# bcaitech1/p4-fr-sorry-math-but-love-you

Measured on NVIDIA B200. Metric: EfficientSATRN greedy-decode images/sec, higher is better.
Workload: dtype bf16

## Files before the change

p4-fr-sorry-math-but-love-you_b200/csrc/kernels_decode_bf16.cu:

```cuda
#include <cooperative_groups.h>
#include <cstdio>
#include <cstdlib>

#include "common.cuh"
#include "kernels.h"

namespace cg = cooperative_groups;

namespace frx {

namespace {

#ifndef FRX_DEC_D
#define FRX_DEC_D 256
#define FRX_DEC_FF 1024
#define FRX_DEC_NAME(x) x
#endif
#ifndef FRX_DEC_HPC
#define FRX_DEC_HPC 1
#endif
#ifndef FRX_DEC_HD
#define FRX_DEC_HD 32
#endif
constexpr int D = FRX_DEC_D;
// ... 136 lines not shown
      mma_bf16(acc[j][1], a1, wk[j].z, wk[j].w);
    }
  };
  if constexpr (C::TOT <= 16) {
    uint4 w[C::TOT];
#pragma unroll
    for (int idx = 0; idx < C::TOT; ++idx) {
      const int kk = idx / C::TPW, j = idx % C::TPW;
      if (idx < PF) w[idx] = pre.w[idx];
      else w[idx] = wload(kk, j);
    }
#pragma unroll
    for (int kk = 0; kk < C::KPW; ++kk) kstep(kk, &w[kk * C::TPW]);
  } else {
    static_assert(PF == 0 || PF == C::TPW, "streaming stages prefetch exactly their first k-pair");
    constexpr int RING = 3;
    uint4 w[RING][C::TPW];
#pragma unroll
    for (int r = 0; r < RING - 1; ++r)
#pragma unroll
      for (int j = 0; j < C::TPW; ++j) {
        if (r < C::KPW) w[r][j] = (PF > 0 && r == 0) ? pre.w[j] : wload(r, j);
      }
#pragma unroll
    for (int kk = 0; kk < C::KPW; ++kk) {
      if (kk + RING - 1 < C::KPW) {
#pragma unroll
        for (int j = 0; j < C::TPW; ++j) w[(kk + RING - 1) % RING][j] = wload(kk + RING - 1, j);
      }
      kstep(kk, w[kk % RING]);
    }
  }
#pragma unroll
  for (int j = 0; j < C::TPW; ++j)
    *reinterpret_cast<float2*>(red + ((size_t)(ks * NT + tg + j * C::TG) * 32 + lane) * 2) =
        make_float2(acc[j][0][0] + acc[j][1][0], acc[j][0][1] + acc[j][1][1]);
  __syncthreads();
  if (threadIdx.x < C::UNITS * C::NSUB) {
    const int u = threadIdx.x % C::UNITS, sub = threadIdx.x / C::UNITS;
    const int tile = u >> 3, row = u & 7;
    float v[8];
#pragma unroll
    for (int i = 0; i < 8; ++i) v[i] = 0.f;
#pragma unroll
    for (int k2 = 0; k2 < KS; ++k2) {
      const float4* src = reinterpret_cast<const float4*>(red + ((size_t)(k2 * NT + tile) * 32 + row * 4) * 2);
      const float4 lo = src[0], hi = src[1];
      v[0] += lo.x; v[1] += lo.y; v[2] += lo.z; v[3] += lo.w;
      v[4] += hi.x; v[5] += hi.y; v[6] += hi.z; v[7] += hi.w;
    }
    epi(tile, row, v, sub);
  }
}

__device__ __forceinline__ uint32_t mapa_u32(uint32_t addr, uint32_t rank) {
  uint32_t r;
  asm volatile("mapa.shared::cluster.u32 %0, %1, %2;\n" : "=r"(r) : "r"(addr), "r"(rank));
  return r;
}
__device__ __forceinline__ void st_async_b32(uint32_t raddr, uint32_t v, uint32_t rbar) {
  asm volatile("st.async.weak.shared::cluster.mbarrier::complete_tx::bytes.b32 [%0], %1, [%2];\n" ::"r"(raddr), "r"(v), "r"(rbar) : "memory");
}
__device__ __forceinline__ void st_async_v4(uint32_t raddr, uint4 v, uint32_t rbar) {
  asm volatile("st.async.weak.shared::cluster.mbarrier::complete_tx::bytes.v4.b32 [%0], {%1, %2, %3, %4}, [%5];\n" ::"r"(raddr), "r"(v.x), "r"(v.y), "r"(v.z), "r"(v.w), "r"(rbar) : "memory");
}
__device__ __forceinline__ void mbar_init(uint32_t bar, uint32_t count) {
  asm volatile("mbarrier.init.shared::cta.b64 [%0], %1;\n" ::"r"(bar), "r"(count) : "memory");
}
__device__ __forceinline__ void mbar_expect_tx(uint32_t bar, uint32_t bytes) {
  asm volatile("mbarrier.arrive.expect_tx.shared::cta.b64 _, [%0], %1;\n" ::"r"(bar), "r"(bytes) : "memory");
}
__device__ __forceinline__ void mbar_wait(uint32_t bar, uint32_t parity) {
  uint32_t ok = 0;
#ifndef FRX_DEC_SPINLIMIT
#define FRX_DEC_SPINLIMIT (1ll << 26)
#endif
#pragma unroll 1
  for (long long spins = 0; spins < FRX_DEC_SPINLIMIT; ++spins) {
    asm volatile(
        "{\n"
        ".reg .pred p;\n"
        "mbarrier.try_wait.parity.shared::cta.b64 p, [%1], %2;\n"
        "selp.u32 %0, 1, 0, p;\n"
        "}\n" : "=r"(ok) : "r"(bar), "r"(parity) : "memory");
    if (ok) return;
  }
  __trap();
}


struct LnParams { float g[D / 32], b[D / 32]; };
__device__ __forceinline__ LnParams load_ln(const float* __restrict__ g, const float* __restrict__ b) {
  LnParams o;
  const int lane = threadIdx.x & 31;
#pragma unroll
  for (int i = 0; i < D / 32; ++i) { o.g[i] = __ldg(g + i * 32 + lane); o.b[i] = __ldg(b + i * 32 + lane); }
  return o;
}

__device__ __forceinline__ void layernorm_rows(Smem& s, const LnParams& P) {
  const int row = threadIdx.x >> 5, lane = threadIdx.x & 31;
  if (row >= NIMG) return;
  float v[D / 32];
#pragma unroll
  for (int i = 0; i < D / 32; ++i) v[i] = s.pre[row][i * 32 + lane];
  const float shift = __shfl_sync(0xffffffffu, v[0], 0);
  float s1 = 0.f, s2 = 0.f;
#pragma unroll
  for (int i = 0; i < D / 32; ++i) { const float d = v[i] - shift; s1 += d; s2 = fmaf(d, d, s2); }
#pragma unroll
  for (int o = 16; o > 0; o >>= 1) {
    s1 += __shfl_xor_sync(0xffffffffu, s1, o);
    s2 += __shfl_xor_sync(0xffffffffu, s2, o);
  }
  const float md = s1 * (1.f / D);
  const float mean = shift + md;
  const float rstd = rsqrtf(fmaxf(s2 * (1.f / D) - md * md, 0.f) + 1e-5f);
#pragma unroll
  for (int i = 0; i < D / 32; ++i) {
    const int c = i * 32 + lane;
    const float o = (v[i] - mean) * rstd * P.g[i] + P.b[i];
    s.xres[row][c] = o;
    s.abf[row][c] = __float2bfloat16_rn(o);
  }
}

struct KVStage { __nv_bfloat16 k[32][HD], v[32][HD]; };

__device__ __forceinline__ int kv_perm(int row) {
  if constexpr (HD == 32) return (row >> 1) & 3;
  else return row & (HD / 8 - 1);
}
__device__ __forceinline__ uint32_t kv_swz(int row, int chunk) { return (uint32_t)(row * (HD * 2) + ((chunk ^ kv_perm(row)) << 4)); }

__device__ __forceinline__ void kv_request(KVStage& st, const __nv_bfloat16* __restrict__ Kc, const __nv_bfloat16* __restrict__ Vc,
                                           int kb, int n_hist, const int* __restrict__ chain) {
  if (kb < n_hist) {
    const int lane = threadIdx.x & 31;
    const uint32_t ks = smem_u32(&st.k[0][0]), vs = smem_u32(&st.v[0][0]);
#pragma unroll
    for (int i = 0; i < HD / 8; ++i) {
      const int id = lane + 32 * i, row = id / (HD / 8), chunk = id % (HD / 8);
      const int key = kb + row;
      const uint32_t bytes = key < n_hist ? 16u : 0u;
      int src = key < n_hist ? key : 0;
      if (chain) src = __ldg(chain + src);
      const size_t off = (size_t)src * HD + ((chunk ^ kv_perm(src)) << 3);
      asm volatile("cp.async.cg.shared.global [%0], [%1], 16, %2;\n" ::"r"(ks + kv_swz(row, chunk)), "l"(Kc + off), "r"(bytes) : "memory");
      asm volatile("cp.async.cg.shared.global [%0], [%1], 16, %2;\n" ::"r"(vs + kv_swz(row, chunk)), "l"(Vc + off), "r"(bytes) : "memory");
    }
  }
  asm volatile("cp.async.commit_group;\n" ::: "memory");
}
__device__ __forceinline__ void kv_request_bulk(KVStage& st, uint32_t bar, const __nv_bfloat16* __restrict__ Kc,
                                                const __nv_bfloat16* __restrict__ Vc, int kb, int n_hist) {
  if (kb < n_hist && (threadIdx.x & 31) == 0) {
    const int rows = n_hist - kb < 32 ? n_hist - kb : 32;
    const uint32_t bytes = (uint32_t)rows * (HD * 2);
    asm volatile("mbarrier.arrive.expect_tx.shared::cta.b64 _, [%0], %1;\n" ::"r"(bar), "r"(2u * bytes) : "memory");
    asm volatile("cp.async.bulk.shared::cluster.global.mbarrier::complete_tx::bytes [%0], [%1], %2, [%3];\n"
                 ::"r"(smem_u32(&st.k[0][0])), "l"(Kc + (size_t)kb * HD), "r"(bytes), "r"(bar) : "memory");
    asm volatile("cp.async.bulk.shared::cluster.global.mbarrier::complete_tx::bytes [%0], [%1], %2, [%3];\n"
                 ::"r"(smem_u32(&st.v[0][0])), "l"(Vc + (size_t)kb * HD), "r"(bytes), "r"(bar) : "memory");
  }
}
__device__ __forceinline__ void kv_prime(KVStage* ring, const __nv_bfloat16* __restrict__ Kc, const __nv_bfloat16* __restrict__ Vc, int n_hist,
                                         const int* __restrict__ chain, uint32_t kvbar) {
  if (!KV_BULK || chain) {
#pragma unroll
    for (int d = 0; d < KVD; ++d) kv_request(ring[d], Kc, Vc, 32 * d, n_hist, chain);
  } else {
#pragma unroll
    for (int d = 0; d < KVD; ++d) kv_request_bulk(ring[d], kvbar + 8u * d, Kc, Vc, 32 * d, n_hist);
  }
}

__device__ __forceinline__ float ex2f(float x) {
  float y;
  asm("ex2.approx.ftz.f32 %0, %1;\n" : "=f"(y) : "f"(x));
  return y;
}

template <bool BULK>
__device__ __forceinline__ void attend_mma(KVStage* ring, const float* __restrict__ q, const __nv_bfloat16* __restrict__ Kc,
                                           const __nv_bfloat16* __restrict__ Vc, int n_hist, const int* __restrict__ chain,
                                           uint32_t kvbar, uint32_t& kvphase, const __nv_bfloat16* __restrict__ kx,
                                           const __nv_bfloat16* __restrict__ vx, float qscale,
                                           float (&o)[HD / 4], long long* pw = nullptr) {
  constexpr int NK = HD / 16;
  constexpr int ND = HD / 8;
  const int lane = threadIdx.x & 31, tig = lane & 3;
  uint32_t aq[NK][4];
#pragma unroll
  for (int ks = 0; ks < NK; ++ks) {
    const float2 qa = *reinterpret_cast<const float2*>(q + 16 * ks + 2 * tig), qb = *reinterpret_cast<const float2*>(q + 16 * ks + 8 + 2 * tig);
    aq[ks][0] = pack_bf16(qa.x * qscale, qa.y * qscale); aq[ks][1] = 0u;
    aq[ks][2] = pack_bf16(qb.x * qscale, qb.y * qscale); aq[ks][3] = 0u;
  }
  float m = -INFINITY, l = 0.f;
  float acc[ND][4];
#pragma unroll
  for (int nt = 0; nt < ND; ++nt)
#pragma unroll
    for (int e = 0; e < 4; ++e) acc[nt][e] = 0.f;
  const int lrow = lane & 7, lmat = lane >> 3;
  uint32_t koff[ND / 4], voff[ND / 2];
#pragma unroll
  for (int c4 = 0; c4 < ND / 4; ++c4) koff[c4] = kv_swz(lrow, 4 * c4 + lmat);
#pragma unroll
  for (int np = 0; np < ND / 2; ++np) voff[np] = kv_swz((lmat & 1) * 8 + lrow, 2 * np + (lmat >> 1));
  int slot = 0;
  for (int kb = 0; kb < n_hist; kb += 32) {
    KVStage& st = ring[slot];
    const int cur = slot;
    slot = slot + 1 == KVD ? 0 : slot + 1;
    const uint32_t ks = smem_u32(&st.k[0][0]), vs = smem_u32(&st.v[0][0]);
    long long tw = 0;
    if (pw) tw = clock64();
    if (!BULK) {
      asm volatile("cp.async.wait_group %0;\n" ::"n"(KVD - 1) : "memory");
    } else {
      mbar_wait(kvbar + 8u * cur, (kvphase >> cur) & 1u);
      kvphase ^= 1u << cur;
    }
    if (pw) { const long long tn = clock64(); pw[0] += tn - tw; pw[1] += 1; tw = tn; }
    __syncwarp();
    uint32_t kf[4][ND], vf[2][ND / 2][4];
#pragma unroll
    for (int j = 0; j < 4; ++j)
#pragma unroll
      for (int c4 = 0; c4 < ND / 4; ++c4)
        asm volatile("ldmatrix.sync.aligned.m8n8.x4.shared.b16 {%0,%1,%2,%3}, [%4];\n"
                     : "=r"(kf[j][4 * c4 + 0]), "=r"(kf[j][4 * c4 + 1]), "=r"(kf[j][4 * c4 + 2]), "=r"(kf[j][4 * c4 + 3])
                     : "r"(ks + koff[c4] + (uint32_t)(j * 8 * HD * 2)));
#pragma unroll
    for (int ks2 = 0; ks2 < 2; ++ks2)
#pragma unroll
      for (int np = 0; np < ND / 2; ++np)
        asm volatile("ldmatrix.sync.aligned.m8n8.x4.trans.shared.b16 {%0,%1,%2,%3}, [%4];\n"
                     : "=r"(vf[ks2][np][0]), "=r"(vf[ks2][np][1]), "=r"(vf[ks2][np][2]), "=r"(vf[ks2][np][3])
                     : "r"(vs + voff[np] + (uint32_t)(ks2 * 16 * HD * 2)));
    __syncwarp();
    if (!BULK) kv_request(st, Kc, Vc, kb + 32 * KVD, n_hist, chain);
    else kv_request_bulk(st, kvbar + 8u * cur, Kc, Vc, kb + 32 * KVD, n_hist);
    if (pw) { const long long tn = clock64(); pw[2] += tn - tw; tw = tn; }
    float sc[4][4];
#pragma unroll
    for (int j = 0; j < 4; ++j) {
#pragma unroll
      for (int e = 0; e < 4; ++e) sc[j][e] = 0.f;
#pragma unroll
      for (int k2 = 0; k2 < NK; ++k2) mma_bf16(sc[j], aq[k2], kf[j][2 * k2], kf[j][2 * k2 + 1]);
    }
    if (!BULK || kb + 32 > n_hist) {
#pragma unroll
      for (int j = 0; j < 4; ++j)
#pragma unroll
        for (int e = 0; e < 2; ++e)
          if (kb + 8 * j + 2 * tig + e >= n_hist) sc[j][e] = -INFINITY;
    }
    float cm = fmaxf(fmaxf(fmaxf(sc[0][0], sc[0][1]), fmaxf(sc[1][0], sc[1][1])), fmaxf(fmaxf(sc[2][0], sc[2][1]), fmaxf(sc[3][0], sc[3][1])));
    cm = fmaxf(cm, __shfl_xor_sync(0xffffffffu, cm, 1));
    cm = fmaxf(cm, __shfl_xor_sync(0xffffffffu, cm, 2));
    cm = fmaxf(cm, m);
    if (!BULK || cm > m) {
      const float scale = ex2f(m - cm);
      m = cm;
      l *= scale;
#pragma unroll
      for (int nt = 0; nt < ND; ++nt) { acc[nt][0] *= scale; acc[nt][1] *= scale; }
    }
    if (pw) { const long long tn = clock64(); pw[3] += tn - tw; tw = tn; }
    float pr[4][2];
#pragma unroll
    for (int j = 0; j < 4; ++j)
#pragma unroll
      for (int e = 0; e < 2; ++e) pr[j][e] = ex2f(sc[j][e] - m);
    l += ((pr[0][0] + pr[0][1]) + (pr[1][0] + pr[1][1])) + ((pr[2][0] + pr[2][1]) + (pr[3][0] + pr[3][1]));
#pragma unroll
    for (int ks2 = 0; ks2 < 2; ++ks2) {
      const uint32_t ap[4] = {pack_bf16(pr[2 * ks2][0], pr[2 * ks2][1]), 0u, pack_bf16(pr[2 * ks2 + 1][0], pr[2 * ks2 + 1][1]), 0u};
#pragma unroll
      for (int np = 0; np < ND / 2; ++np) {
        mma_bf16(acc[2 * np], ap, vf[ks2][np][0], vf[ks2][np][1]);
        mma_bf16(acc[2 * np + 1], ap, vf[ks2][np][2], vf[ks2][np][3]);
      }
    }
    if (pw) pw[4] += clock64() - tw;
  }
  l += __shfl_xor_sync(0xffffffffu, l, 1);
  l += __shfl_xor_sync(0xffffffffu, l, 2);
  if (kx) {
    constexpr int DPT = HD / 4;
    float part = 0.f;
#pragma unroll
    for (int c8 = 0; c8 < DPT / 8; ++c8) {
      const float4 q0 = *reinterpret_cast<const float4*>(q + DPT * tig + 8 * c8), q1 = *reinterpret_cast<const float4*>(q + DPT * tig + 8 * c8 + 4);
      float kf[8];
      unpack8(*reinterpret_cast<const uint4*>(kx + DPT * tig + 8 * c8), kf);
      part += q0.x * kf[0] + q0.y * kf[1] + q0.z * kf[2] + q0.w * kf[3] + q1.x * kf[4] + q1.y * kf[5] + q1.z * kf[6] + q1.w * kf[7];
    }
    part += __shfl_xor_sync(0xffffffffu, part, 1);
    part += __shfl_xor_sync(0xffffffffu, part, 2);
    const float s_cur = part * qscale;
    const float M = fmaxf(m, s_cur);
    const float gs = ex2f(m - M);
    const float pc = ex2f(s_cur - M);
    l = l * gs + pc;
#pragma unroll
    for (int nt = 0; nt < ND; ++nt) {
      const __nv_bfloat162 v2 = *reinterpret_cast<const __nv_bfloat162*>(vx + 8 * nt + 2 * tig);
      acc[nt][0] = fmaf(pc, __low2float(v2), acc[nt][0] * gs);
      acc[nt][1] = fmaf(pc, __high2float(v2), acc[nt][1] * gs);
    }
  }
  const float inv = __fdividef(1.f, l);
#pragma unroll
  for (int nt = 0; nt < ND; ++nt) { o[2 * nt] = acc[nt][0] * inv; o[2 * nt + 1] = acc[nt][1] * inv; }
}

__device__ __forceinline__ float4 ldg4(const float* p) { return __ldg(reinterpret_cast<const float4*>(p)); }

__device__ __noinline__ int sift_pick(const float* lrow, int V, int4* state, const int* __restrict__ flags, const int* __restrict__ limit,
                                      SiftIds ids, float* prow) {
  const int lane = threadIdx.x & 31;
  const int4 stt = *state;
  float mx = -INFINITY;
  for (int i = lane; i < V; i += 32) mx = fmaxf(mx, lrow[i]);
#pragma unroll
  for (int o = 16; o > 0; o >>= 1) mx = fmaxf(mx, __shfl_xor_sync(0xffffffffu, mx, o));
  float sum = 0.f;
  for (int i = lane; i < V; i += 32) sum += expf(lrow[i] - mx);
#pragma unroll
  for (int o = 16; o > 0; o >>= 1) sum += __shfl_xor_sync(0xffffffffu, sum, o);
  const int cur = stt.x;
  const int cf = (cur >= 0 && cur < V) ? __ldg(flags + cur) : 0;
  const int clim = (cur >= 0 && cur < V) ? __ldg(limit + cur) : 0;
  float best = -INFINITY;
  int bi = 0x7fffffff;
  for (int i = lane; i < V; i += 32) {
    bool black = (i == ids.sos) || (i == ids.empty) || (i == ids.rbrace && stt.z == stt.w);
    if (cur == ids.eos) {
    } else if (cur == ids.sos) {
      black = black || (__ldg(flags + i) & 1);
    } else if (cf & 2) {
      black = black || (i != ids.underbar);
    } else if (cf & 4) {
      black = black || (i != ids.lbrace);
    } else {
      if ((cf & 8) && i == ids.underbar) black = true;
      if ((cf & 16) && i == ids.lbrace) black = true;
      if (clim > 0 && stt.y >= clim && i == cur) black = true;
    }
    const float pv = black ? 0.f : expf(lrow[i] - mx) / sum;
    if (prow) prow[i] = pv;
    if (pv > best) { best = pv; bi = i; }
  }
#pragma unroll
  for (int o = 16; o > 0; o >>= 1) {
    const float ob = __shfl_xor_sync(0xffffffffu, best, o);
    const int oi = __shfl_xor_sync(0xffffffffu, bi, o);
    if (ob > best || (ob == best && oi < bi)) { best = ob; bi = oi; }
  }
  if (bi < 0 || bi >= V) bi = 0;
  __syncwarp();
  if (lane == 0) {
    int4 n = stt;
    n.y = (bi == stt.x) ? stt.y + 1 : 1;
    if (bi == ids.lbrace) n.z += 1;
    else if (bi == ids.rbrace) n.w += 1;
    n.x = bi;
    *state = n;
  }
  __syncwarp();
  return bi;
}
struct Bias8 { float4 a, b; };
__device__ __forceinline__ Bias8 ldg_bias8(const float* p, bool active) {
  Bias8 o;
  o.a = o.b = make_float4(0.f, 0.f, 0.f, 0.f);
  if (active) { o.a = ldg4(p); o.b = ldg4(p + 4); }
  return o;
}

}

#ifndef FRX_DEC_MINBLOCKS
#define FRX_DEC_MINBLOCKS (NTHR <= 256 ? 2 : 1)
#endif
__global__ void __cluster_dims__(CL, 1, 1) __launch_bounds__(NTHR, FRX_DEC_MINBLOCKS)
FRX_DEC_NAME(dec_cluster_bf16_kernel)(const DecClusterP p) {
  extern __shared__ __align__(16) unsigned char smem_raw[];
  Smem& s = *reinterpret_cast<Smem*>(smem_raw);
  cg::cluster_group cl = cg::this_cluster();
  const int r = (int)cl.block_rank();
  const int img0 = p.img_base + (blockIdx.x / CL) * NIMG;
  const int tid = threadIdx.x, warp = tid >> 5, lane = tid & 31;
  const uint64_t pol = make_evict_last_policy();
  const float qscale = 1.4426950408889634f / sqrtf((float)D);
  const float emb_scale = sqrtf((float)D);
  const int L = p.L, T = p.T, V = p.V, B = p.B;
  constexpr int LDA = D + APAD, LDA2 = FF + APAD;
  constexpr int KPD = D / 32, KPF = FF / 32;
  constexpr size_t WT = (size_t)KPD * 32;
  constexpr int KS = 2;
  constexpr int PF_A = GC<NTA, KPD, KS>::TOT > 16 ? GC<NTA, KPD, KS>::TPW : (GC<NTA, KPD, KS>::TOT < 6 ? GC<NTA, KPD, KS>::TOT : 6);
  constexpr int PF_S = GC<NTS, KPD, KS>::TOT;
  constexpr int PF_E = GC<NTE, KPD, KS>::TOT < 8 ? GC<NTE, KPD, KS>::TOT : 8;
  constexpr int PF_F = GC<NTS, KPF, KS>::TOT < 8 ? GC<NTS, KPF, KS>::TOT : 8;

  if (tid == 0) {
#pragma unroll
    for (int l = 0; l < 4; ++l) s.lw[l] = p.layer[l];
  }
  for (int i = tid; i < NIMG * D; i += NTHR) {
    const int row = i / D, c = i % D;
    const int b = min(img0 + row, p.B - 1);
    long long tok = p.sos;
    if (p.first_tok32) tok = __ldg(p.first_tok32 + b);
    else if (p.first_tok64) tok = __ldg(p.first_tok64 + b);
    const int pos0 = p.hist_len ? __ldg(p.hist_len + b) : 0;
    float v = __ldg(p.emb + (size_t)tok * D + c) * emb_scale + __ldg(p.pe + (size_t)pos0 * D + c);
    s.xres[row][c] = v;
    s.abf[row][c] = __float2bfloat16_rn(v);
  }
  if (tid < NIMG) s.sift[tid] = make_int4(p.sift_ids.sos, 1, 0, 0);
  const uint32_t bar0 = smem_u32(&s.bar[0]), bar1 = smem_u32(&s.bar[1]);
  if (tid == 0) {
    mbar_init(bar0, 1);
    mbar_init(bar1, 1);
    asm volatile("fence.mbarrier_init.release.cluster;\n" ::: "memory");
  }
  if (KV_BULK) {
    if (lane == 0) {
#pragma unroll
      for (int d = 0; d < KVD; ++d) mbar_init(smem_u32(&s.kvbar[warp][d]), 1);
    }
    for (int i = tid; i < (int)(sizeof(s.kvst) / 16); i += NTHR) reinterpret_cast<uint4*>(&s.kvst[0][0][0][0][0])[i] = make_uint4(0u, 0u, 0u, 0u);
    asm volatile("fence.proxy.async.shared::cta;\n" ::: "memory");
  }
  __syncthreads();
  cl.sync();
  int gstage = 0;
  auto stage_bar = [&]() -> uint32_t { return (gstage & 1) ? bar1 : bar0; };
  auto stage_begin = [&](uint32_t bytes) { if (tid == 0) mbar_expect_tx(stage_bar(), bytes); };
  auto stage_end = [&]() { mbar_wait(stage_bar(), (uint32_t)((gstage >> 1) & 1)); ++gstage; };
  int rsel = 0;
  auto next_red = [&]() -> float* { rsel ^= 1; return s.red[rsel]; };
  float* const logit_s = reinterpret_cast<float*>(&s.abf2[0][0]);
  constexpr int LGS = VP + FPAD;
  static_assert(NIMG * LGS * 4 <= NIMG * (FF + APAD) * 2, "the fp32 logits view must fit in abf2");

  const bool profiling = p.prof != nullptr && blockIdx.x == 0 && tid == 0;
  if (profiling) for (int i = 0; i < 16; ++i) s.prof[i] = 0;
  long long tprev = clock64();
  auto mark = [&](int id) {
    if (profiling) {
      long long now = clock64();
      s.prof[id] += now - tprev;
      tprev = now;
    }
  };
  const int wimg = warp % NIMG, whc = warp / NIMG;
  const int head = r * HPC + whc;
  const int b_mine = img0 + wimg;
  const bool mine = b_mine < B;
  const int hist0 = (mine && p.hist_len) ? __ldg(p.hist_len + b_mine) : 0;
  const int* const chain = (mine && p.chain) ? p.chain + (size_t)b_mine * T : nullptr;
  KVStage* const kvst = reinterpret_cast<KVStage*>(&s.kvst[warp][0][0][0][0]);
  const uint32_t kvbar = smem_u32(&s.kvbar[warp][0]);
  uint32_t kvphase = 0;

  auto store_attn = [&](uint32_t sb, const float (&o)[HD / 4]) {
    const uint32_t dst = (uint32_t)(lane >> 2);
    if (dst < (uint32_t)CL) {
      const uint32_t rb = mapa_u32(sb, dst);
      const uint32_t la = mapa_u32(smem_u32(&s.obf[wimg][head * HD + 2 * (lane & 3)]), dst);
#pragma unroll
      for (int nt = 0; nt < HD / 8; ++nt) st_async_b32(la + nt * 16, pack_bf16(o[2 * nt], o[2 * nt + 1]), rb);
    }
  };
  auto pre_bias = [&](const float* bias) {
    return ldg_bias8(bias + r * SW + ((tid % (NTS * 8)) >> 3) * 8, true);
  };
  auto pre_epi = [&](uint32_t sb, const Bias8& bias, bool relu) {
    return [&, sb, bias, relu](int tile, int row, float (&v)[8], int sub) {
      constexpr int NSUB_S = GC<NTS, KPD, KS>::NSUB, DPT = (CL + NSUB_S - 1) / NSUB_S;
      if (sub * DPT >= CL) return;
      const int col = r * SW + tile * 8;
      const float4 b0 = bias.a, b1 = bias.b;
      const float4 x0 = *reinterpret_cast<const float4*>(&s.xres[row][col]), x1 = *reinterpret_cast<const float4*>(&s.xres[row][col + 4]);
      float o[8] = {v[0] + b0.x, v[1] + b0.y, v[2] + b0.z, v[3] + b0.w, v[4] + b1.x, v[5] + b1.y, v[6] + b1.z, v[7] + b1.w};
      if (relu) {
#pragma unroll
        for (int i = 0; i < 8; ++i) o[i] = fmaxf(o[i], 0.f);
      }
      const uint4 lo = make_uint4(__float_as_uint(o[0] + x0.x), __float_as_uint(o[1] + x0.y), __float_as_uint(o[2] + x0.z), __float_as_uint(o[3] + x0.w));
      const uint4 hi = make_uint4(__float_as_uint(o[4] + x1.x), __float_as_uint(o[5] + x1.y), __float_as_uint(o[6] + x1.z), __float_as_uint(o[7] + x1.w));
#pragma unroll
      for (int d = 0; d < DPT; ++d) {
        const uint32_t dst = (uint32_t)(sub * DPT + d);
        if (dst >= (uint32_t)CL) break;
        const uint32_t la = mapa_u32(smem_u32(&s.pre[row][col]), dst), rb = mapa_u32(sb, dst);
        st_async_v4(la, lo, rb);
        st_async_v4(la + 16, hi, rb);
      }
    };
  };
  auto qkv_bias = [&](const float* bias) {
    const int tile = tid >> 3, seg = tile / NTS, wc = (tile % NTS) * 8;
    return ldg_bias8(bias + seg * D + r * SW + wc, tid < NTA * 8);
  };
  auto qkv_epi = [&](const Bias8& bias) {
    return [&, bias](int tile, int row, float (&v)[8], int sub) {
      if (sub != 0) return;
      const int seg = tile / NTS, wc = (tile % NTS) * 8, hc = wc / HD, col = wc % HD;
      const float4 b0 = bias.a, b1 = bias.b;
      const float o[8] = {v[0] + b0.x, v[1] + b0.y, v[2] + b0.z, v[3] + b0.w, v[4] + b1.x, v[5] + b1.y, v[6] + b1.z, v[7] + b1.w};
      if (seg == 0) {
        *reinterpret_cast<float4*>(&s.qh[hc][row][col]) = make_float4(o[0], o[1], o[2], o[3]);
        *reinterpret_cast<float4*>(&s.qh[hc][row][col + 4]) = make_float4(o[4], o[5], o[6], o[7]);
      } else {
        __nv_bfloat16(*dst)[HD + APAD] = seg == 1 ? s.kcur[hc] : s.vcur[hc];
        *reinterpret_cast<uint4*>(&dst[row][col]) =
            make_uint4(pack_bf16(o[0], o[1]), pack_bf16(o[2], o[3]), pack_bf16(o[4], o[5]), pack_bf16(o[6], o[7]));
      }
    };
  };
  auto cache_rows = [&](int lc, int t, const uint4* wp, const float* bias) {
    const Bias8 cb = ldg_bias8(bias + ((tid >> 3) / NTS) * D + r * SW + ((tid >> 3) % NTS) * 8, tid < NTC * 8);
    gemm2<NTC, KPD, KS>(next_red(), &s.abf[0][0], LDA, wp, pol, WPre<0>{}, [&](int tile, int row, float (&v)[8], int sub) {
      const int b = img0 + row;
      if (sub != 0 || b >= B) return;
      const int seg = tile / NTS, wc = (tile % NTS) * 8, hd = r * HPC + wc / HD, col = wc % HD;
      const float4 b0 = cb.a, b1 = cb.b;
      __nv_bfloat16* dst = seg == 0 ? p.kself : p.vself;
      const int wrow = (p.slot ? __ldg(p.slot + b) : (p.hist_len ? __ldg(p.hist_len + b) : 0)) + t;
      *reinterpret_cast<uint4*>(dst + (((((size_t)lc * B + b) * H + hd) * T) + wrow) * HD + (((col >> 3) ^ kv_perm(wrow)) << 3)) =
          make_uint4(pack_bf16(v[0] + b0.x, v[1] + b0.y), pack_bf16(v[2] + b0.z, v[3] + b0.w),
                     pack_bf16(v[4] + b1.x, v[5] + b1.y), pack_bf16(v[6] + b1.z, v[7] + b1.w));
      if (KV_BULK) asm volatile("fence.proxy.async.global;\n" ::: "memory");
    });
  };

  auto pre_a = prefetch_w<NTA, KPD, KS, PF_A>(p.w_first + (size_t)r * NTA * WT, pol);
  auto prime_self = [&](int l, int t) {
    const size_t base = ((((size_t)l * B + (mine ? b_mine : 0)) * H + head) * T) * HD;
    kv_prime(kvst, p.kself + base, p.vself + base, mine ? hist0 + t : 0, chain, kvbar);
  };
  auto prime_cross = [&](int l) {
    const size_t base = ((((size_t)l * B + (mine ? b_mine : 0)) * H + head) * p.S) * HD;
    kv_prime(kvst, p.kcross + base, p.vcross + base, mine ? p.S : 0, nullptr, kvbar);
  };
  prime_self(0, 0);
  bool self_primed = true;
  for (int t = 0; t < p.steps; ++t) {
    for (int l = 0; l < L; ++l) {
      const DecClusterLayer& W = s.lw[l];
      {
        const size_t base = ((((size_t)l * B + (mine ? b_mine : 0)) * H + head) * T) * HD;
        const int n_hist = mine ? hist0 + t : 0;
        if (!self_primed) prime_self(l, t);
        self_primed = false;
        const uint4* wp = l == 0 ? p.w_first + (size_t)r * NTA * WT : s.lw[l - 1].w_next + ((size_t)r * (NTC + NTA) + NTC) * WT;
        const Bias8 bias = qkv_bias(l == 0 ? p.b_first : s.lw[l - 1].b_next + 2 * D);
        gemm2<NTA, KPD, KS>(next_red(), &s.abf[0][0], LDA, wp, pol, pre_a, qkv_epi(bias));
        __syncthreads();
        mark(0);
        stage_begin(NIMG * D * 2u);
        const uint32_t sb = stage_bar();
        float o[HD / 4];
        if (!KV_BULK || chain)
          attend_mma<false>(kvst, &s.qh[whc][wimg][0], p.kself + base, p.vself + base, n_hist, chain, kvbar, kvphase, &s.kcur[whc][wimg][0], &s.vcur[whc][wimg][0], qscale, o,
                            profiling ? &s.prof[11] : nullptr);
        else
          attend_mma<true>(kvst, &s.qh[whc][wimg][0], p.kself + base, p.vself + base, n_hist, nullptr, kvbar, kvphase, &s.kcur[whc][wimg][0], &s.vcur[whc][wimg][0], qscale, o,
                           profiling ? &s.prof[11] : nullptr);
        store_attn(sb, o);
        if (EARLY_PRIME) prime_cross(l);
        mark(1);
      }
      const auto pre_b = prefetch_w<NTS, KPD, KS, PF_S>(W.w_o + (size_t)r * NTS * WT, pol);
      const Bias8 bias_b = pre_bias(W.b_o);
      if (l > 0) cache_rows(l - 1, t, s.lw[l - 1].w_next + (size_t)r * (NTC + NTA) * WT, s.lw[l - 1].b_next);
      mark(2);
      stage_end();
      mark(3);
      stage_begin(NIMG * D * 4u);
      gemm2<NTS, KPD, KS>(next_red(), &s.obf[0][0], LDA, W.w_o + (size_t)r * NTS * WT, pol, pre_b, pre_epi(stage_bar(), bias_b, false));
      mark(4);
      const LnParams lnp1 = load_ln(W.ln1_g, W.ln1_b);
      const auto pre_c = prefetch_w<NTS, KPD, KS, PF_S>(W.w_q2 + (size_t)r * NTS * WT, pol);
      const Bias8 bias_c = ldg_bias8(W.b_q2 + r * SW + (tid >> 3) * 8, tid < NTS * 8);
      stage_end();
      mark(5);
      layernorm_rows(s, lnp1);
      __syncthreads();
      mark(6);
      {
        const size_t base = ((((size_t)l * B + (mine ? b_mine : 0)) * H + head) * p.S) * HD;
        const int n_keys = mine ? p.S : 0;
        if (!EARLY_PRIME) prime_cross(l);
        gemm2<NTS, KPD, KS>(next_red(), &s.abf[0][0], LDA, W.w_q2 + (size_t)r * NTS * WT, pol, pre_c,
                          [&](int tile, int row, float (&v)[8], int sub) {
                            if (sub != 0) return;
                            const int wc = tile * 8, hc = wc / HD, col = wc % HD;
                            const float4 b0 = bias_c.a, b1 = bias_c.b;
                            *reinterpret_cast<float4*>(&s.qh[hc][row][col]) = make_float4(v[0] + b0.x, v[1] + b0.y, v[2] + b0.z, v[3] + b0.w);
                            *reinterpret_cast<float4*>(&s.qh[hc][row][col + 4]) = make_float4(v[4] + b1.x, v[5] + b1.y, v[6] + b1.z, v[7] + b1.w);
                          });
        __syncthreads();
        mark(4);
        stage_begin(NIMG * D * 2u);
        const uint32_t sb = stage_bar();
        float o[HD / 4];
        if (mine) {
          attend_mma<KV_BULK>(kvst, &s.qh[whc][wimg][0], p.kcross + base, p.vcross + base, n_keys, nullptr, kvbar, kvphase, nullptr, nullptr, qscale, o);
        } else {
#pragma unroll
          for (int i = 0; i < HD / 4; ++i) o[i] = 0.f;
        }
        store_attn(sb, o);
        if (EARLY_PRIME) {
          if (l + 1 < L) { prime_self(l + 1, t); self_primed = true; }
          else if (L >= 2 && t + 1 < p.steps) { prime_self(0, t + 1); self_primed = true; }
        }
        mark(7);
      }
      const auto pre_d = prefetch_w<NTS, KPD, KS, PF_S>(W.w_o2 + (size_t)r * NTS * WT, pol);
      const Bias8 bias_d = pre_bias(W.b_o2);
      stage_end();
      mark(3);
      stage_begin(NIMG * D * 4u);
      gemm2<NTS, KPD, KS>(next_red(), &s.obf[0][0], LDA, W.w_o2 + (size_t)r * NTS * WT, pol, pre_d, pre_epi(stage_bar(), bias_d, false));
      mark(4);
      const LnParams lnp2 = load_ln(W.ln2_g, W.ln2_b);
      const auto pre_e = prefetch_w<NTE, KPD, KS, PF_E>(W.w_f0 + (size_t)r * NTE * WT, pol);
      const Bias8 bias_e = ldg_bias8(W.b_f0 + r * FS + ((tid % (NTE * 8)) >> 3) * 8, true);
      stage_end();
      mark(5);
      layernorm_rows(s, lnp2);
      __syncthreads();
      mark(6);
      {
        stage_begin(NIMG * FF * 2u);
        const uint32_t sb = stage_bar();
        gemm2<NTE, KPD, KS>(next_red(), &s.abf[0][0], LDA, W.w_f0 + (size_t)r * NTE * WT, pol, pre_e,
                           [&](int tile, int row, float (&v)[8], int sub) {
                             const int col = r * FS + tile * 8;
                             const float4 b0 = bias_e.a, b1 = bias_e.b;
                             const uint4 o = make_uint4(pack_bf16(fmaxf(v[0] + b0.x, 0.f), fmaxf(v[1] + b0.y, 0.f)),
                                                        pack_bf16(fmaxf(v[2] + b0.z, 0.f), fmaxf(v[3] + b0.w, 0.f)),
                                                        pack_bf16(fmaxf(v[4] + b1.x, 0.f), fmaxf(v[5] + b1.y, 0.f)),
                                                        pack_bf16(fmaxf(v[6] + b1.z, 0.f), fmaxf(v[7] + b1.w, 0.f)));
                             const uint32_t la = smem_u32(&s.abf2[row][col]);
                             constexpr int NSUB_E = GC<NTE, KPD, KS>::NSUB, DPT = (CL + NSUB_E - 1) / NSUB_E;
#pragma unroll
                             for (int d = 0; d < DPT; ++d) {
                               const uint32_t dst = (uint32_t)(sub * DPT + d);
                               if (dst < (uint32_t)CL) st_async_v4(mapa_u32(la, dst), o, mapa_u32(sb, dst));
                             }
                           });
        mark(8);
      }
      const auto pre_f = prefetch_w<NTS, KPF, KS, PF_F>(W.w_f1 + (size_t)r * NTS * KPF * 32, pol);
      const Bias8 bias_f = pre_bias(W.b_f1);
      stage_end();
      mark(5);
      stage_begin(NIMG * D * 4u);
      gemm2<NTS, KPF, KS>(next_red(), &s.abf2[0][0], LDA2, W.w_f1 + (size_t)r * NTS * KPF * 32, pol, pre_f, pre_epi(stage_bar(), bias_f, true));
      mark(9);
      const LnParams lnp3 = load_ln(W.ln3_g, W.ln3_b);
      const bool last_layer = l + 1 >= L;
      constexpr int PF_G = GC<NG, KPD, KS>::TOT;
      WPre<PF_G> pre_g;
      float gbias[8];
#pragma unroll
      for (int i = 0; i < 8; ++i) gbias[i] = 0.f;
      if (!last_layer) pre_a = prefetch_w<NTA, KPD, KS, PF_A>(W.w_next + ((size_t)r * (NTC + NTA) + NTC) * WT, pol);
      else {
        pre_g = prefetch_w<NG, KPD, KS, PF_G>(W.w_next + ((size_t)r * (NTC + NG) + NTC) * WT, pol);
        const int col = r * (VP / CL) + ((tid % (NG * 8)) >> 3) * 8;
        const float* gb = W.b_next + 2 * D;
        if (tid < NG * 8 * CL) {
#pragma unroll
          for (int i = 0; i < 8; ++i) gbias[i] = col + i < V ? __ldg(gb + col + i) : 0.f;
        }
      }
      stage_end();
      mark(5);
      layernorm_rows(s, lnp3);
      __syncthreads();
      mark(6);
      if (last_layer) {
        stage_begin(NIMG * VP * 4u);
        const uint32_t sb = stage_bar();
        gemm2<NG, KPD, KS>(next_red(), &s.abf[0][0], LDA, W.w_next + ((size_t)r * (NTC + NG) + NTC) * WT, pol, pre_g,
                          [&](int tile, int row, float (&v)[8], int sub) {
                            constexpr int NSUB_G = GC<NG, KPD, KS>::NSUB, DPT = (CL + NSUB_G - 1) / NSUB_G;
                            if (sub * DPT >= CL) return;
                            const int col = r * (VP / CL) + tile * 8;
#pragma unroll
                            for (int i = 0; i < 8; ++i) v[i] += gbias[i];
#pragma unroll
                            for (int d = 0; d < DPT; ++d) {
                              const uint32_t dst = (uint32_t)(sub * DPT + d);
                              if (dst >= (uint32_t)CL) break;
                              const uint32_t la = mapa_u32(smem_u32(logit_s + row * LGS + col), dst), rb = mapa_u32(sb, dst);
                              st_async_v4(la, make_uint4(__float_as_uint(v[0]), __float_as_uint(v[1]), __float_as_uint(v[2]), __float_as_uint(v[3])), rb);
                              st_async_v4(la + 16, make_uint4(__float_as_uint(v[4]), __float_as_uint(v[5]), __float_as_uint(v[6]), __float_as_uint(v[7])), rb);
                            }
                            const int b = img0 + row;
                            if (sub == (CL > 1 ? 1 : 0) && p.logits && b < B && !p.sift_flags) {
                              float* lp = p.logits + ((size_t)b * p.steps + t) * V + col;
#pragma unroll
                              for (int i = 0; i < 8; ++i)
                                if (col + i < V) lp[i] = v[i];
                            }
                          });
        mark(4);
        pre_a = prefetch_w<NTA, KPD, KS, PF_A>(p.w_first + (size_t)r * NTA * WT, pol);
        cache_rows(l, t, W.w_next + (size_t)r * (NTC + NG) * WT, W.b_next);
        mark(2);
        stage_end();
        mark(5);
      }
    }
    if (warp < NIMG) {
      const int row = warp;
      int bi;
      if (p.sift_flags) {
        float* prow = (mine && r == 0 && p.logits) ? p.logits + ((size_t)b_mine * p.steps + t) * V : nullptr;
        bi = sift_pick(logit_s + row * LGS, V, &s.sift[row], p.sift_flags, p.sift_limit, p.sift_ids, prow);
      } else {
        float best = -INFINITY;
        bi = 0x7fffffff;
        for (int i = lane; i < V; i += 32) {
          float v = logit_s[row * LGS + i];
          if (v > best) { best = v; bi = i; }
        }
#pragma unroll
        for (int o = 16; o > 0; o >>= 1) {
          float ob = __shfl_xor_sync(0xffffffffu, best, o);
          int oi = __shfl_xor_sync(0xffffffffu, bi, o);
          if (ob > best || (ob == best && oi < bi)) { best = ob; bi = oi; }
        }
        if (bi < 0 || bi >= V) bi = 0;
      }
      int nxt = bi;
      if (mine) {
        if (p.forced) nxt = (int)p.forced[(size_t)b_mine * p.steps + t];
        if (r == 0 && lane == 0 && p.tokens) p.tokens[(size_t)b_mine * p.steps + t] = bi;
      }
      if (t + 1 < p.steps) {
        const float* pe = p.pe + (size_t)(hist0 + t + 1) * D;
#pragma unroll
        for (int i = 0; i < D / 32; ++i) {
          const int c = i * 32 + lane;
          float v = __ldg(p.emb + (size_t)nxt * D + c) * emb_scale + __ldg(pe + c);
          s.xres[row][c] = v;
          s.abf[row][c] = __float2bfloat16_rn(v);
        }
      }
    }
    __syncthreads();
    mark(10);
  }
  cl.sync();
  if (profiling) for (int i = 0; i < 16; ++i) p.prof[i] = s.prof[i];
}

size_t FRX_DEC_NAME(dec_cluster_smem_bytes)() { return sizeof(Smem); }

// ... 61 lines not shown
```

Baseline: 13020.

## Transpose decode attention MMA so keys fill the M dimension, not padded query rows

Attention now puts keys and the head dimension in the MMA M dimension with the single query as the N operand, replacing the old layout where the query took the A operand with half its rows zero-padded. Softmax reductions, probability repacking through shuffles and prmt, and the output store layout are rebuilt to match. The KV ring loop is unrolled over the stage count so stage addresses are compile-time constants. The aim is to cut wasted MMA work and register use per KV tile, at the cost of extra shuffles and permutes, and the per-section clock profiling is removed.

```diff
diff --git a/p4-fr-sorry-math-but-love-you_b200/csrc/kernels_decode_bf16.cu b/p4-fr-sorry-math-but-love-you_b200/csrc/kernels_decode_bf16.cu
--- a/p4-fr-sorry-math-but-love-you_b200/csrc/kernels_decode_bf16.cu
+++ b/p4-fr-sorry-math-but-love-you_b200/csrc/kernels_decode_bf16.cu
@@ -312,16 +312,16 @@
   }
   asm volatile("cp.async.commit_group;\n" ::: "memory");
 }
-__device__ __forceinline__ void kv_request_bulk(KVStage& st, uint32_t bar, const __nv_bfloat16* __restrict__ Kc,
+__device__ __forceinline__ void kv_request_bulk(uint32_t ks, uint32_t bar, const __nv_bfloat16* __restrict__ Kc,
                                                 const __nv_bfloat16* __restrict__ Vc, int kb, int n_hist) {
   if (kb < n_hist && (threadIdx.x & 31) == 0) {
     const int rows = n_hist - kb < 32 ? n_hist - kb : 32;
     const uint32_t bytes = (uint32_t)rows * (HD * 2);
     asm volatile("mbarrier.arrive.expect_tx.shared::cta.b64 _, [%0], %1;\n" ::"r"(bar), "r"(2u * bytes) : "memory");
     asm volatile("cp.async.bulk.shared::cluster.global.mbarrier::complete_tx::bytes [%0], [%1], %2, [%3];\n"
-                 ::"r"(smem_u32(&st.k[0][0])), "l"(Kc + (size_t)kb * HD), "r"(bytes), "r"(bar) : "memory");
+                 ::"r"(ks), "l"(Kc + (size_t)kb * HD), "r"(bytes), "r"(bar) : "memory");
     asm volatile("cp.async.bulk.shared::cluster.global.mbarrier::complete_tx::bytes [%0], [%1], %2, [%3];\n"
-                 ::"r"(smem_u32(&st.v[0][0])), "l"(Vc + (size_t)kb * HD), "r"(bytes), "r"(bar) : "memory");
+                 ::"r"(ks + 32u * HD * 2u), "l"(Vc + (size_t)kb * HD), "r"(bytes), "r"(bar) : "memory");
   }
 }
 __device__ __forceinline__ void kv_prime(KVStage* ring, const __nv_bfloat16* __restrict__ Kc, const __nv_bfloat16* __restrict__ Vc, int n_hist,
@@ -331,7 +331,7 @@
     for (int d = 0; d < KVD; ++d) kv_request(ring[d], Kc, Vc, 32 * d, n_hist, chain);
   } else {
 #pragma unroll
-    for (int d = 0; d < KVD; ++d) kv_request_bulk(ring[d], kvbar + 8u * d, Kc, Vc, 32 * d, n_hist);
+    for (int d = 0; d < KVD; ++d) kv_request_bulk(smem_u32(&ring[d]), kvbar + 8u * d, Kc, Vc, 32 * d, n_hist);
   }
 }
 
@@ -339,6 +339,12 @@
   float y;
   asm("ex2.approx.ftz.f32 %0, %1;\n" : "=f"(y) : "f"(x));
   return y;
+}
+
+__device__ __forceinline__ uint32_t prmt(uint32_t a, uint32_t b, uint32_t sel) {
+  uint32_t r;
+  asm("prmt.b32 %0, %1, %2, %3;\n" : "=r"(r) : "r"(a), "r"(b), "r"(sel));
+  return r;
 }
 
 template <bool BULK>
@@ -346,110 +352,108 @@
                                            const __nv_bfloat16* __restrict__ Vc, int n_hist, const int* __restrict__ chain,
                                            uint32_t kvbar, uint32_t& kvphase, const __nv_bfloat16* __restrict__ kx,
                                            const __nv_bfloat16* __restrict__ vx, float qscale,
-                                           float (&o)[HD / 4], long long* pw = nullptr) {
+                                           float (&o)[HD / 8]) {
   constexpr int NK = HD / 16;
-  constexpr int ND = HD / 8;
-  const int lane = threadIdx.x & 31, tig = lane & 3;
-  uint32_t aq[NK][4];
+  constexpr int NM = HD / 16;
+  constexpr uint32_t STAGE = sizeof(KVStage), VOFF = 32u * HD * 2u, TILE = 16u * HD * 2u;
+  const int lane = threadIdx.x & 31, g = lane >> 2, tig = lane & 3;
+  const uint32_t ring0 = smem_u32(ring);
+  uint32_t bq[NK][2];
 #pragma unroll
   for (int ks = 0; ks < NK; ++ks) {
     const float2 qa = *reinterpret_cast<const float2*>(q + 16 * ks + 2 * tig), qb = *reinterpret_cast<const float2*>(q + 16 * ks + 8 + 2 * tig);
-    aq[ks][0] = pack_bf16(qa.x * qscale, qa.y * qscale); aq[ks][1] = 0u;
-    aq[ks][2] = pack_bf16(qb.x * qscale, qb.y * qscale); aq[ks][3] = 0u;
+    bq[ks][0] = pack_bf16(qa.x * qscale, qa.y * qscale);
+    bq[ks][1] = pack_bf16(qb.x * qscale, qb.y * qscale);
   }
   float m = -INFINITY, l = 0.f;
-  float acc[ND][4];
-#pragma unroll
-  for (int nt = 0; nt < ND; ++nt)
-#pragma unroll
-    for (int e = 0; e < 4; ++e) acc[nt][e] = 0.f;
+  float acc[NM][4];
+#pragma unroll
+  for (int mt = 0; mt < NM; ++mt)
+#pragma unroll
+    for (int e = 0; e < 4; ++e) acc[mt][e] = 0.f;
   const int lrow = lane & 7, lmat = lane >> 3;
-  uint32_t koff[ND / 4], voff[ND / 2];
-#pragma unroll
-  for (int c4 = 0; c4 < ND / 4; ++c4) koff[c4] = kv_swz(lrow, 4 * c4 + lmat);
-#pragma unroll
-  for (int np = 0; np < ND / 2; ++np) voff[np] = kv_swz((lmat & 1) * 8 + lrow, 2 * np + (lmat >> 1));
-  int slot = 0;
-  for (int kb = 0; kb < n_hist; kb += 32) {
-    KVStage& st = ring[slot];
-    const int cur = slot;
-    slot = slot + 1 == KVD ? 0 : slot + 1;
-    const uint32_t ks = smem_u32(&st.k[0][0]), vs = smem_u32(&st.v[0][0]);
-    long long tw = 0;
-    if (pw) tw = clock64();
-    if (!BULK) {
-      asm volatile("cp.async.wait_group %0;\n" ::"n"(KVD - 1) : "memory");
-    } else {
-      mbar_wait(kvbar + 8u * cur, (kvphase >> cur) & 1u);
-      kvphase ^= 1u << cur;
-    }
-    if (pw) { const long long tn = clock64(); pw[0] += tn - tw; pw[1] += 1; tw = tn; }
-    __syncwarp();
-    uint32_t kf[4][ND], vf[2][ND / 2][4];
-#pragma unroll
-    for (int j = 0; j < 4; ++j)
-#pragma unroll
-      for (int c4 = 0; c4 < ND / 4; ++c4)
-        asm volatile("ldmatrix.sync.aligned.m8n8.x4.shared.b16 {%0,%1,%2,%3}, [%4];\n"
-                     : "=r"(kf[j][4 * c4 + 0]), "=r"(kf[j][4 * c4 + 1]), "=r"(kf[j][4 * c4 + 2]), "=r"(kf[j][4 * c4 + 3])
-                     : "r"(ks + koff[c4] + (uint32_t)(j * 8 * HD * 2)));
-#pragma unroll
-    for (int ks2 = 0; ks2 < 2; ++ks2)
-#pragma unroll
-      for (int np = 0; np < ND / 2; ++np)
-        asm volatile("ldmatrix.sync.aligned.m8n8.x4.trans.shared.b16 {%0,%1,%2,%3}, [%4];\n"
-                     : "=r"(vf[ks2][np][0]), "=r"(vf[ks2][np][1]), "=r"(vf[ks2][np][2]), "=r"(vf[ks2][np][3])
-                     : "r"(vs + voff[np] + (uint32_t)(ks2 * 16 * HD * 2)));
-    __syncwarp();
-    if (!BULK) kv_request(st, Kc, Vc, kb + 32 * KVD, n_hist, chain);
-    else kv_request_bulk(st, kvbar + 8u * cur, Kc, Vc, kb + 32 * KVD, n_hist);
-    if (pw) { const long long tn = clock64(); pw[2] += tn - tw; tw = tn; }
-    float sc[4][4];
-#pragma unroll
-    for (int j = 0; j < 4; ++j) {
-#pragma unroll
-      for (int e = 0; e < 4; ++e) sc[j][e] = 0.f;
-#pragma unroll
-      for (int k2 = 0; k2 < NK; ++k2) mma_bf16(sc[j], aq[k2], kf[j][2 * k2], kf[j][2 * k2 + 1]);
-    }
-    if (!BULK || kb + 32 > n_hist) {
-#pragma unroll
-      for (int j = 0; j < 4; ++j)
-#pragma unroll
-        for (int e = 0; e < 2; ++e)
-          if (kb + 8 * j + 2 * tig + e >= n_hist) sc[j][e] = -INFINITY;
-    }
-    float cm = fmaxf(fmaxf(fmaxf(sc[0][0], sc[0][1]), fmaxf(sc[1][0], sc[1][1])), fmaxf(fmaxf(sc[2][0], sc[2][1]), fmaxf(sc[3][0], sc[3][1])));
-    cm = fmaxf(cm, __shfl_xor_sync(0xffffffffu, cm, 1));
-    cm = fmaxf(cm, __shfl_xor_sync(0xffffffffu, cm, 2));
-    cm = fmaxf(cm, m);
-    if (!BULK || cm > m) {
-      const float scale = ex2f(m - cm);
-      m = cm;
-      l *= scale;
-#pragma unroll
-      for (int nt = 0; nt < ND; ++nt) { acc[nt][0] *= scale; acc[nt][1] *= scale; }
-    }
-    if (pw) { const long long tn = clock64(); pw[3] += tn - tw; tw = tn; }
-    float pr[4][2];
-#pragma unroll
-    for (int j = 0; j < 4; ++j)
-#pragma unroll
-      for (int e = 0; e < 2; ++e) pr[j][e] = ex2f(sc[j][e] - m);
-    l += ((pr[0][0] + pr[0][1]) + (pr[1][0] + pr[1][1])) + ((pr[2][0] + pr[2][1]) + (pr[3][0] + pr[3][1]));
-#pragma unroll
-    for (int ks2 = 0; ks2 < 2; ++ks2) {
-      const uint32_t ap[4] = {pack_bf16(pr[2 * ks2][0], pr[2 * ks2][1]), 0u, pack_bf16(pr[2 * ks2 + 1][0], pr[2 * ks2 + 1][1]), 0u};
-#pragma unroll
-      for (int np = 0; np < ND / 2; ++np) {
-        mma_bf16(acc[2 * np], ap, vf[ks2][np][0], vf[ks2][np][1]);
-        mma_bf16(acc[2 * np + 1], ap, vf[ks2][np][2], vf[ks2][np][3]);
-      }
-    }
-    if (pw) pw[4] += clock64() - tw;
-  }
-  l += __shfl_xor_sync(0xffffffffu, l, 1);
-  l += __shfl_xor_sync(0xffffffffu, l, 2);
+  uint32_t koff[NK], voff[NM];
+#pragma unroll
+  for (int ks = 0; ks < NK; ++ks) koff[ks] = kv_swz((lmat & 1) * 8 + lrow, 2 * ks + (lmat >> 1));
+#pragma unroll
+  for (int mt = 0; mt < NM; ++mt) voff[mt] = VOFF + kv_swz((lmat >> 1) * 8 + lrow, 2 * mt + (lmat & 1));
+  const int src0 = 8 * tig, src1 = 8 * tig + 4;
+  for (int kb0 = 0; kb0 < n_hist; kb0 += 32 * KVD) {
+#pragma unroll
+    for (int d = 0; d < KVD; ++d) {
+      const int kb = kb0 + 32 * d;
+      if (KVD > 1 && kb >= n_hist) break;
+      const uint32_t st = ring0 + d * STAGE;
+      if (!BULK) {
+        asm volatile("cp.async.wait_group %0;\n" ::"n"(KVD - 1) : "memory");
+      } else {
+        mbar_wait(kvbar + 8u * d, (kvphase >> d) & 1u);
+        kvphase ^= 1u << d;
+      }
+      __syncwarp();
+      uint32_t kf[2][NK][4], vf[NM][2][4];
+#pragma unroll
+      for (int mt = 0; mt < 2; ++mt)
+#pragma unroll
+        for (int ks = 0; ks < NK; ++ks)
+          asm volatile("ldmatrix.sync.aligned.m8n8.x4.shared.b16 {%0,%1,%2,%3}, [%4];\n"
+                       : "=r"(kf[mt][ks][0]), "=r"(kf[mt][ks][1]), "=r"(kf[mt][ks][2]), "=r"(kf[mt][ks][3])
+                       : "r"(st + koff[ks] + mt * TILE));
+#pragma unroll
+      for (int mt = 0; mt < NM; ++mt)
+#pragma unroll
+        for (int ks2 = 0; ks2 < 2; ++ks2)
+          asm volatile("ldmatrix.sync.aligned.m8n8.x4.trans.shared.b16 {%0,%1,%2,%3}, [%4];\n"
+                       : "=r"(vf[mt][ks2][0]), "=r"(vf[mt][ks2][1]), "=r"(vf[mt][ks2][2]), "=r"(vf[mt][ks2][3])
+                       : "r"(st + voff[mt] + ks2 * TILE));
+      __syncwarp();
+      if (!BULK) kv_request(ring[d], Kc, Vc, kb + 32 * KVD, n_hist, chain);
+      else kv_request_bulk(st, kvbar + 8u * d, Kc, Vc, kb + 32 * KVD, n_hist);
+      float sc[2][4];
+#pragma unroll
+      for (int mt = 0; mt < 2; ++mt) {
+#pragma unroll
+        for (int e = 0; e < 4; ++e) sc[mt][e] = 0.f;
+#pragma unroll
+        for (int ks = 0; ks < NK; ++ks) mma_bf16(sc[mt], kf[mt][ks], bq[ks][0], bq[ks][1]);
+      }
+      float sv[4] = {sc[0][0], sc[0][2], sc[1][0], sc[1][2]};
+      if (!BULK || kb + 32 > n_hist) {
+#pragma unroll
+        for (int i = 0; i < 4; ++i)
+          if (kb + 8 * i + g >= n_hist) sv[i] = -INFINITY;
+      }
+      float cm = fmaxf(fmaxf(sv[0], sv[1]), fmaxf(sv[2], sv[3]));
+      cm = fmaxf(cm, __shfl_xor_sync(0xffffffffu, cm, 4));
+      cm = fmaxf(cm, __shfl_xor_sync(0xffffffffu, cm, 8));
+      cm = fmaxf(cm, __shfl_xor_sync(0xffffffffu, cm, 16));
+      cm = fmaxf(cm, m);
+      if (!BULK || cm > m) {
+        const float scale = ex2f(m - cm);
+        m = cm;
+        l *= scale;
+#pragma unroll
+        for (int mt = 0; mt < NM; ++mt) { acc[mt][0] *= scale; acc[mt][2] *= scale; }
+      }
+      float pr[4];
+#pragma unroll
+      for (int i = 0; i < 4; ++i) pr[i] = ex2f(sv[i] - m);
+      float nb[4];
+#pragma unroll
+      for (int i = 0; i < 4; ++i) nb[i] = __shfl_xor_sync(0xffffffffu, pr[i], 4);
+      l += ((pr[0] + nb[0]) + (pr[1] + nb[1])) + ((pr[2] + nb[2]) + (pr[3] + nb[3]));
+#pragma unroll
+      for (int ks2 = 0; ks2 < 2; ++ks2) {
+        const uint32_t x = pack_bf16(pr[2 * ks2], pr[2 * ks2 + 1]);
+        const uint32_t x0 = __shfl_sync(0xffffffffu, x, src0), x1 = __shfl_sync(0xffffffffu, x, src1);
+        const uint32_t b0 = prmt(x0, x1, 0x5410u), b1 = prmt(x0, x1, 0x7632u);
+#pragma unroll
+        for (int mt = 0; mt < NM; ++mt) mma_bf16(acc[mt], vf[mt][ks2], b0, b1);
+      }
+    }
+  }
+  l += __shfl_xor_sync(0xffffffffu, l, 8);
+  l += __shfl_xor_sync(0xffffffffu, l, 16);
   if (kx) {
     constexpr int DPT = HD / 4;
     float part = 0.f;
@@ -468,15 +472,14 @@
     const float pc = ex2f(s_cur - M);
     l = l * gs + pc;
 #pragma unroll
-    for (int nt = 0; nt < ND; ++nt) {
-      const __nv_bfloat162 v2 = *reinterpret_cast<const __nv_bfloat162*>(vx + 8 * nt + 2 * tig);
-      acc[nt][0] = fmaf(pc, __low2float(v2), acc[nt][0] * gs);
-      acc[nt][1] = fmaf(pc, __high2float(v2), acc[nt][1] * gs);
+    for (int mt = 0; mt < NM; ++mt) {
+      acc[mt][0] = fmaf(pc, __bfloat162float(vx[16 * mt + g]), acc[mt][0] * gs);
+      acc[mt][2] = fmaf(pc, __bfloat162float(vx[16 * mt + 8 + g]), acc[mt][2] * gs);
     }
   }
   const float inv = __fdividef(1.f, l);
 #pragma unroll
-  for (int nt = 0; nt < ND; ++nt) { o[2 * nt] = acc[nt][0] * inv; o[2 * nt + 1] = acc[nt][1] * inv; }
+  for (int mt = 0; mt < NM; ++mt) { o[2 * mt] = acc[mt][0] * inv; o[2 * mt + 1] = acc[mt][2] * inv; }
 }
 
 __device__ __forceinline__ float4 ldg4(const float* p) { return __ldg(reinterpret_cast<const float4*>(p)); }
@@ -631,13 +634,23 @@
   const uint32_t kvbar = smem_u32(&s.kvbar[warp][0]);
   uint32_t kvphase = 0;
 
-  auto store_attn = [&](uint32_t sb, const float (&o)[HD / 4]) {
-    const uint32_t dst = (uint32_t)(lane >> 2);
+  auto store_attn = [&](uint32_t sb, const float (&o)[HD / 8]) {
+    const int g = lane >> 2;
+    uint32_t w[HD / 8];
+#pragma unroll
+    for (int mt = 0; mt < HD / 16; ++mt) {
+      const uint32_t mine_p = pack_bf16(o[2 * mt], o[2 * mt + 1]);
+      const uint32_t nb_p = __shfl_xor_sync(0xffffffffu, mine_p, 4);
+      const uint32_t lo = (g & 1) ? nb_p : mine_p, hi = (g & 1) ? mine_p : nb_p;
+      w[2 * mt] = prmt(lo, hi, 0x5410u);
+      w[2 * mt + 1] = prmt(lo, hi, 0x7632u);
+    }
+    const uint32_t dst = (uint32_t)((g & 1) * 4 + (lane & 3));
     if (dst < (uint32_t)CL) {
       const uint32_t rb = mapa_u32(sb, dst);
-      const uint32_t la = mapa_u32(smem_u32(&s.obf[wimg][head * HD + 2 * (lane & 3)]), dst);
-#pragma unroll
-      for (int nt = 0; nt < HD / 8; ++nt) st_async_b32(la + nt * 16, pack_bf16(o[2 * nt], o[2 * nt + 1]), rb);
+      const uint32_t la = mapa_u32(smem_u32(&s.obf[wimg][head * HD + (g & ~1)]), dst);
+#pragma unroll
+      for (int i = 0; i < HD / 8; ++i) st_async_b32(la + (i >> 1) * 32 + (i & 1) * 16, w[i], rb);
     }
   };
   auto pre_bias = [&](const float* bias) {
@@ -729,13 +742,11 @@
         mark(0);
         stage_begin(NIMG * D * 2u);
         const uint32_t sb = stage_bar();
-        float o[HD / 4];
+        float o[HD / 8];
         if (!KV_BULK || chain)
-          attend_mma<false>(kvst, &s.qh[whc][wimg][0], p.kself + base, p.vself + base, n_hist, chain, kvbar, kvphase, &s.kcur[whc][wimg][0], &s.vcur[whc][wimg][0], qscale, o,
-                            profiling ? &s.prof[11] : nullptr);
+          attend_mma<false>(kvst, &s.qh[whc][wimg][0], p.kself + base, p.vself + base, n_hist, chain, kvbar, kvphase, &s.kcur[whc][wimg][0], &s.vcur[whc][wimg][0], qscale, o);
         else
-          attend_mma<true>(kvst, &s.qh[whc][wimg][0], p.kself + base, p.vself + base, n_hist, nullptr, kvbar, kvphase, &s.kcur[whc][wimg][0], &s.vcur[whc][wimg][0], qscale, o,
-                           profiling ? &s.prof[11] : nullptr);
+          attend_mma<true>(kvst, &s.qh[whc][wimg][0], p.kself + base, p.vself + base, n_hist, nullptr, kvbar, kvphase, &s.kcur[whc][wimg][0], &s.vcur[whc][wimg][0], qscale, o);
         store_attn(sb, o);
         if (EARLY_PRIME) prime_cross(l);
         mark(1);
@@ -773,12 +784,12 @@
         mark(4);
         stage_begin(NIMG * D * 2u);
         const uint32_t sb = stage_bar();
-        float o[HD / 4];
+        float o[HD / 8];
         if (mine) {
           attend_mma<KV_BULK>(kvst, &s.qh[whc][wimg][0], p.kcross + base, p.vcross + base, n_keys, nullptr, kvbar, kvphase, nullptr, nullptr, qscale, o);
         } else {
 #pragma unroll
-          for (int i = 0; i < HD / 4; ++i) o[i] = 0.f;
+          for (int i = 0; i < HD / 8; ++i) o[i] = 0.f;
         }
         store_attn(sb, o);
         if (EARLY_PRIME) {
```

After: 13180 (median of 6 runs). 1.01x the previous value.
